# Nyrox/raymond

Measured on AMD Instinct MI355X. Metric: Msamples/s (whole node) + achieved HBM GB/s, 1920x1080 @ 500spp 5-bounce, higher is better.
Workload: dtype f64

## Files before the change

### raymond_amd/csrc/api.cpp

```cpp
#define RMD_WITH_HIP 1
#include <algorithm>
#include <cmath>
#include <limits>
#include <cstdio>
#include <cstdlib>
#include <cstring>
#include <new>

#include "internal.hpp"
#include "launch.hpp"

using rmd::bind;

namespace {
thread_local std::string tl_last_error;

rmd_status context_create(int32_t device, hipStream_t stream, bool own_stream, rmd_context **out) {
	if (!out) return rmd::fail(nullptr, RMD_ERR_INVALID_ARGUMENT, "rmd_context_create: null out pointer");
	*out = nullptr;
	int count = 0;
	hipError_t e = hipGetDeviceCount(&count);
	if (e != hipSuccess || count <= 0)
		return rmd::fail(nullptr, RMD_ERR_NO_DEVICE, std::string("no HIP device: ") + (e != hipSuccess ? hipGetErrorString(e) : "device count is 0"));
	if (device < 0 || device >= count) return rmd::fail(nullptr, RMD_ERR_INVALID_ARGUMENT, "rmd_context_create: device ordinal out of range");
// ... 580 lines not shown
		if (k > sample_count / 4u) k = sample_count / 4u;
		may_buffer_unsplit = false;
	} else if (n_wave_tiles != 0) {
		const uint32_t waves_per_slot = has_grid ? 256u : 24u;
		k = (waves_per_slot * ctx->wave_slots + n_wave_tiles - 1u) / n_wave_tiles;
		if (has_grid && k < 2u) k = 2u;
		uint32_t min_samples = has_grid ? (sample_count <= rmd::kChainMaxSamples && ctx->tunable[RMD_TUNE_CHAIN_ITEMS] != 1 ? 2u : rmd::kSplitMinSamplesGrid) : 64u;
		if (ctx->tunable[RMD_TUNE_SPLIT_MIN_SAMPLES] > 0) min_samples = (uint32_t)std::min<int64_t>(ctx->tunable[RMD_TUNE_SPLIT_MIN_SAMPLES], 1 << 20);
		if (k > sample_count / min_samples) k = sample_count / min_samples;
		if (has_grid && k < 2u && sample_count >= 4u && ctx->tunable[RMD_TUNE_SPLIT_MIN_SAMPLES] <= 0) k = 2u;
	}
	if (k > 64u) k = 64u;
	while (k > 1u && (uint64_t)n_wave_tiles * k > 0x7FFFFFFFull) k--;
	if (k < 2u) k = 1u;
	if (buffered) *buffered = k > 1u || may_buffer_unsplit;
	return k;
}

static rmd_status render_tiles_async_impl(rmd_context *ctx, const rmd_scene *scene, const rmd_camera *camera, const rmd_settings *settings,
                                          const rmd_tile_rect *tiles, uint32_t n_tiles, double *accum_dev, double *accum_sq_dev) {
	if (rmd_status s = bind(ctx)) return s;
	if (rmd_status s = check_render_args(ctx, scene, camera, settings)) return s;
	if (!accum_dev || (n_tiles && !tiles)) return rmd::fail(ctx, RMD_ERR_INVALID_ARGUMENT, "rmd_render_tiles: null tiles/accum pointer");
	if (rmd_status s = prepare_wave_tiles(ctx, camera, tiles, n_tiles)) return s;
	if (settings->bounce_limit == 0u) {
		RMD_HIP(ctx, hipEventRecord(ctx->ev_start, ctx->stream));
		RMD_HIP(ctx, hipEventRecord(ctx->ev_stop, ctx->stream));
		ctx->timed = true;
		return RMD_OK;
	}
	rmd::RenderParams P = rmd::make_params(ctx, scene, camera, settings);
	P.n_work = ctx->n_wave_tiles;
	if (P.debug_flags & 24u) {
		RMD_HIP(ctx, ctx->debug_counters.grow(40 * sizeof(unsigned long long)));
		RMD_HIP(ctx, hipMemsetAsync(ctx->debug_counters.as<void>(), 0, 40 * sizeof(unsigned long long), ctx->stream));
		P.debug_counters = ctx->debug_counters.as<unsigned long long>();
	}
	bool buffered = false;
	uint32_t split = choose_split(ctx, scene->n_grids != 0, P.n_work, P.sample_count, &buffered);
	const bool persistent = ctx->tunable[RMD_TUNE_LAUNCH_FORM] != 1;
	if (persistent) RMD_HIP(ctx, ctx->work_counter.grow(256));
	uint32_t per_pass = P.sample_count;
	if (buffered) {
		const size_t bytes_per_sample = (size_t)P.n_work * 64u * rmd::kSampleStride * sizeof(double);
		size_t cap;
		if (ctx->tunable[RMD_TUNE_SCRATCH_CAP_MB] > 0) cap = (size_t)ctx->tunable[RMD_TUNE_SCRATCH_CAP_MB] << 20;
		else {
			size_t free_b = 0, total_b = 0;
			RMD_HIP(ctx, hipMemGetInfo(&free_b, &total_b));
			cap = (free_b + ctx->sample_buf.bytes()) / 8;
		}
		if (bytes_per_sample * per_pass > cap) per_pass = (uint32_t)(cap / bytes_per_sample);
		const uint64_t sectors_per_sample = (uint64_t)P.n_work * 64u;
		if (sectors_per_sample * per_pass > 0xFFFFFFFFull) per_pass = (uint32_t)(0xFFFFFFFFull / sectors_per_sample);
		if (per_pass < 8u) per_pass = 8u;
		if (per_pass > P.sample_count) per_pass = P.sample_count;
		if (sectors_per_sample * per_pass > 0xFFFFFFFFull) split = 1u, buffered = false, per_pass = P.sample_count;
		while (buffered && bytes_per_sample * per_pass > ctx->sample_buf.bytes()) {
			rmd::DeviceBuffer fresh;
			const hipError_t e = fresh.alloc(bytes_per_sample * per_pass);
			if (e == hipSuccess) {
				ctx->sample_buf = std::move(fresh);
				break;
			}
			(void)hipGetLastError();
			if (e != hipErrorOutOfMemory) return rmd::fail(ctx, RMD_ERR_HIP, std::string("hipMalloc(sample scratch): ") + hipGetErrorString(e));
			if (per_pass <= 8u) {
				split = 1u, buffered = false, per_pass = P.sample_count;
// ... 22 lines not shown
			RMD_HIP(ctx, hipMemsetAsync(ctx->work_counter.as<void>(), 0, sizeof(uint32_t), ctx->stream));
			Q.work_counter = ctx->work_counter.as<uint32_t>();
		}
		if (persistent_pass && buffered && scene->n_grids != 0u && ctx->tunable[RMD_TUNE_PATH_QUEUES] != 1) {
			const size_t wave_bytes = rmd::path_queue_bytes_host(rmd::kQueuePaths), need = wave_bytes * ctx->wave_slots;
			if (ctx->queue_buf.bytes() < need) {
				const hipError_t qe = (ctx->debug_flags & 256u) ? hipErrorOutOfMemory : ctx->queue_buf.grow(need);
				if (qe == hipSuccess) {
					RMD_HIP(ctx, hipMemsetAsync(ctx->queue_buf.as<void>(), 0, need, ctx->stream));
				} else {
					(void)hipGetLastError();
					if (qe != hipErrorOutOfMemory) return rmd::fail(ctx, RMD_ERR_HIP, std::string("hipMalloc(path queues): ") + hipGetErrorString(qe));
				}
			}
			if (ctx->queue_buf.bytes()) Q.queue_buf = ctx->queue_buf.as<unsigned char>(), Q.queue_wave_bytes = (uint32_t)wave_bytes, Q.queue_paths = rmd::kQueuePaths;
		}
		if (buffered && scene->n_grids == 0) {
			RMD_HIP(ctx, ctx->tile_done.grow((size_t)P.n_work * sizeof(uint32_t)));
			RMD_HIP(ctx, hipMemsetAsync(ctx->tile_done.as<void>(), 0, (size_t)P.n_work * sizeof(uint32_t), ctx->stream));
			Q.tile_done = ctx->tile_done.as<uint32_t>();
		}
		rmd::LaunchShape shape;
		RMD_HIP(ctx, rmd::launch_render_tiles(ctx->stream, Q, scene->d_objects, scene->d_grids, ctx->wave_tiles.as<rmd::WaveTile>(), accum_dev, persistent_pass ? ctx->n_cus : 0u, &shape,
		                                      accum_sq_dev));
		ctx->last_launch.passes++, ctx->last_launch.split_k = Q.split_k, ctx->last_launch.buffered = Q.buffered;
		ctx->last_launch.persistent = shape.persistent, ctx->last_launch.waves_per_workgroup = shape.waves_per_wg;
		ctx->last_launch.queued = shape.queued;
		ctx->last_launch.chained = shape.chained;
		if (settings->sample_count == 0) break;
	}
	RMD_HIP(ctx, hipEventRecord(ctx->ev_stop, ctx->stream));
	ctx->timed = true;
	if (P.debug_flags & 24u) {
		unsigned long long h[40];
		RMD_HIP(ctx, hipMemcpyAsync(h, ctx->debug_counters.as<void>(), sizeof(h), hipMemcpyDeviceToHost, ctx->stream));
		RMD_HIP(ctx, hipStreamSynchronize(ctx->stream));
		if ((P.debug_flags & 16u) && ctx->last_launch.queued) {
			static const char *kinds[3] = {"GEN  ", "SHADE", "WALK "};
			for (int k = 0; k < 3; k++)
				std::fprintf(stderr, "[rmd queued stamps, cycles] %s trips=%llu fetch=%llu make_ray=%llu simple=%llu walk=%llu ray_push=%llu classify=%llu stores=%llu\n", kinds[k], h[k * 8 + 7],
				             h[k * 8 + 0], h[k * 8 + 1], h[k * 8 + 2], h[k * 8 + 3], h[k * 8 + 4], h[k * 8 + 5], h[k * 8 + 6]);
			std::fprintf(stderr, "[rmd queued stamps, cycles] inside the walks: init=%llu stepping=%llu entry_wait=%llu scan=%llu (chunk search+load+test)=%llu hits=%llu tail=%llu\n",
			             h[24], h[25], h[26], h[27], h[29], h[30], h[31]);
		} else if (P.debug_flags & 16u)
			std::fprintf(stderr, "[rmd stamps, cycles] wave_total=%llu next_ray=%llu simple=%llu walk=%llu classify=%llu | walk: init=%llu stepping=%llu entry_wait=%llu scan=%llu (chunk search+load+test)=%llu hits=%llu tail=%llu\n",
			             h[0], h[1], h[2], h[3], h[4], h[8], h[9], h[10], h[11], h[13], h[14], h[15]);
		else
			std::fprintf(stderr, "[rmd debug] walk_calls=%llu walkers=%llu calls_with_walkers=%llu rounds=%llu wave_steps=%llu lane_steps=%llu test_rounds=%llu tests=%llu chunks=%llu | main_iterations=%llu live_lanes=%llu lanes_with_ray=%llu | stepping iterations with <= 4 / 8 / 16 lanes: %llu / %llu / %llu, with <= 8 lanes while tests wait: %llu\n",
			             h[0], h[1], h[2], h[3], h[4], h[5], h[6], h[8], h[9], h[10], h[11], h[12], h[7], h[13], h[14], h[15]);
		if ((P.debug_flags & 16u) == 0u)
			std::fprintf(stderr, "[rmd debug] sphere pre-test: pairs passed=%llu full chunks=%llu | pairs dropped that pass the reference's test (flag 64; must be 0)=%llu\n", h[17], h[18], h[16]);
		if ((P.debug_flags & 16u) == 0u && (P.debug_flags & 512u))
			std::fprintf(stderr, "[rmd debug] primary candidates: lanes checked=%llu sphere turns left out=%llu trips with two axis pairs left out=%llu | cleared spheres that register a hit (must be 0)=%llu closest hits that differ from the full visit's (must be 0)=%llu\n",
			             h[32], h[35], h[36], h[33], h[34]);
		if ((P.debug_flags & 16u) == 0u && ctx->last_launch.queued)
			std::fprintf(stderr, "[rmd debug] path queues: rays pushed=%llu (of them walks put aside=%llu) rays held in their lanes=%llu hits pushed=%llu hits held in their lanes=%llu\n", h[19], h[22], h[23], h[20], h[21]);
	}
	return RMD_OK;
}

rmd_status rmd_render_tiles_async(rmd_context *ctx, const rmd_scene *scene, const rmd_camera *camera, const rmd_settings *settings,
                                  const rmd_tile_rect *tiles, uint32_t n_tiles, double *accum_dev) {
	return rmd::guarded(ctx, "rmd_render_tiles", [&] { return render_tiles_async_impl(ctx, scene, camera, settings, tiles, n_tiles, accum_dev, nullptr); });
}

rmd_status rmd_render_tiles_moments_async(rmd_context *ctx, const rmd_scene *scene, const rmd_camera *camera, const rmd_settings *settings,
                                          const rmd_tile_rect *tiles, uint32_t n_tiles, double *accum_dev, double *accum_sq_dev) {
	if (accum_sq_dev != nullptr && accum_sq_dev == accum_dev)
		return rmd::fail(ctx, RMD_ERR_INVALID_ARGUMENT, "rmd_render_tiles_moments: accum_sq_dev must not alias accum_dev");
	return rmd::guarded(ctx, "rmd_render_tiles_moments",
	                    [&] { return render_tiles_async_impl(ctx, scene, camera, settings, tiles, n_tiles, accum_dev, accum_sq_dev); });
}

rmd_status rmd_context_set_tunable(rmd_context *ctx, uint32_t key, int64_t value) {
	if (!ctx) return rmd::fail(nullptr, RMD_ERR_INVALID_ARGUMENT, "rmd_context_set_tunable: null context");
	if (key >= RMD_TUNE_COUNT || value < 0) return rmd::fail(ctx, RMD_ERR_INVALID_ARGUMENT, "rmd_context_set_tunable: unknown key or negative value");
	if (key == RMD_TUNE_LAUNCH_FORM && value > 2) return rmd::fail(ctx, RMD_ERR_INVALID_ARGUMENT, "rmd_context_set_tunable: launch form is 0 .. 2");
	ctx->tunable[key] = value;
	return RMD_OK;
}
rmd_status rmd_context_get_tunable(const rmd_context *ctx, uint32_t key, int64_t *out_value) {
	if (!ctx || !out_value || key >= RMD_TUNE_COUNT) return rmd::fail(nullptr, RMD_ERR_INVALID_ARGUMENT, "rmd_context_get_tunable: bad argument");
	*out_value = ctx->tunable[key];
	return RMD_OK;
}

rmd_status rmd_context_memory_info(rmd_context *ctx, uint64_t *out_free_bytes, uint64_t *out_total_bytes) {
// ... 294 lines not shown
```

### raymond_amd/csrc/device_core.hpp

```cpp
#pragma once
#include <hip/hip_runtime.h>
#include <stdint.h>

#include "device_types.hpp"

#define RMD_DEV __device__ __forceinline__
#ifndef RMD_OPT_BITOP3
#if defined(__gfx950__) || !defined(__HIP_DEVICE_COMPILE__)
#define RMD_OPT_BITOP3 1
#else
#define RMD_OPT_BITOP3 0
#endif
#endif
#define RMD_GLOBAL __attribute__((address_space(1)))
template <class T>
__device__ __forceinline__ const RMD_GLOBAL T *as_global(const T *p) {
	return (const RMD_GLOBAL T *)p;
}

namespace rmd {

struct V3 {
	double x, y, z;
};
// ... 337 lines not shown
	st = sqrt64((1.0 - sr) * (1.0 + sr));
}

RMD_DEV void cosine_hemisphere(double r1, double r2, V3 &dir, double &pdf) {
	double sr = sqrt64(r1);
	double phi = 2.0 * kPi * r2;
	pdf = sr;
	double st, ct, sp, cp;
	hemisphere_sincos(sr, st, ct);
	sincos_cw(phi, sp, cp);
	dir = mk(st * cp, ct, st * sp);
}
RMD_DEV V3 importance_sample_ggx(V3 reflect, double roughness, double r1, double r2) {
	double a = roughness * roughness;
	double phi = 2.0 * kPi * r1;
	double theta = a * sqrt64(r2 / (1.0 - r2));
	double st, ct, sp, cp;
	sincos_cw(theta, st, ct);
	sincos_cw(phi, sp, cp);
	V3 h = mk(st * cp, ct, st * sp);
	V3 tg, bt;
	onb(reflect, tg, bt);
	return normalize(mat3_mul(tg, reflect, bt, h));
}

RMD_DEV double pow5(double x) {
	const double x2 = x * x;
	const double x4 = x2 * x2;
	return x4 * x;
}
RMD_DEV V3 sel(bool c, V3 a, V3 b) { return mk(c ? a.x : b.x, c ? a.y : b.y, c ? a.z : b.z); }

#define RMD_UNDEF(v) asm volatile("" : "=v"(v));
struct NextRayShadeIn {
	V3 normal, frag, color;
	double roughness, metal;
};
RMD_DEV void next_ray(const RenderParams &P, bool do_shade, bool do_prim, const NextRayShadeIn &in, V3 cam_pos, uint32_t prim_x, uint32_t prim_y, Rng &rng,
                      V3 &ro, V3 &rd, V3 &T) {
	const bool gen = do_shade || do_prim;
	double u_first, u_second;
	RMD_UNDEF(u_first) RMD_UNDEF(u_second)
	const double r = (double)rng.lobe_bits * (1.0 / 4194304.0);
	if (gen) {
		uint32_t w0, w1, w2, w3;
		philox4x32_10(rng.pixel, rng.sample, rng.block, 0u, P.key0, P.key1, w0, w1, w2, w3);
		rng.block++;
		u_first = Rng::to_unit(w0, w1), u_second = Rng::to_unit(w2, w3);
		rng.lobe_bits = Rng::spare22(w0, w2);
	}
	V3 pre, view, f0;
	RMD_UNDEF(pre.x) RMD_UNDEF(pre.y) RMD_UNDEF(pre.z) RMD_UNDEF(view.x) RMD_UNDEF(view.y) RMD_UNDEF(view.z) RMD_UNDEF(f0.x) RMD_UNDEF(f0.y) RMD_UNDEF(f0.z)
	bool diffuse = false;
	double prob_d, pdf_d;
	RMD_UNDEF(prob_d) RMD_UNDEF(pdf_d)
	if (do_shade) {
		const V3 normal = in.normal;
		view = normalize(cam_pos - in.frag);
		f0 = mk(lerp(0.04, in.color.x, in.metal), lerp(0.04, in.color.y, in.metal), lerp(0.04, in.color.z, in.metal));
		const double r1 = u_first, r2 = u_second;
		prob_d = lerp(0.5, 0.0, in.metal);
		diffuse = r < prob_d;
		double phi, st, ct, sp, cp;
		V3 axis;
		double root_arg = r1;
		if (!diffuse) root_arg = div_lean(r2, 1.0 - r2);
		const double root = sqrt64(root_arg);
		if (diffuse) {
			hemisphere_sincos(root, st, ct);
			phi = 2.0 * kPi * r2;
			pdf_d = root;
			axis = normal;
		} else {
			const double a = in.roughness * in.roughness;
			phi = 2.0 * kPi * r1;
			sincos_cw(a * root, st, ct);
			axis = normalize(-view - 2.0 * (-dot(view, normal) * normal));
		}
		sincos_cw(phi, sp, cp);
		const V3 local = mk(st * cp, ct, st * sp);
		V3 tg, bt;
		onb(axis, tg, bt);
		pre = mat3_mul(tg, axis, bt, local);
	}
	if (do_prim) {
		const double x = (double)prim_x + (u_first - 0.5);
		const double y = (double)prim_y + (u_second - 0.5);
		const double sx = P.inv_width == P.inv_width ? div_by(x + 0.5, P.width, P.inv_width) : (x + 0.5) / P.width;
		const double sy = P.inv_height == P.inv_height ? div_by(y + 0.5, P.height, P.inv_height) : (y + 0.5) / P.height;
		pre = mk((2.0 * sx - 1.0) * P.tan_half_fov * P.aspect, (1.0 - 2.0 * sy) * P.tan_half_fov, 1.0);
	}
	V3 sw = pre;
	if (gen) sw = normalize(pre);
	if (do_prim) {
		ro = cam_pos, rd = sw;
// ... 9 lines not shown
		V3 vec;
		double N, Dn;
		if (diffuse) {
			const V3 diffuse_part = (mk(1.0, 1.0, 1.0) - F) * (1.0 - in.metal);
			vec = hadamard(diffuse_part, in.color);
			N = fmax(n_dot_sw, 0.0);
			Dn = prob_d * pdf_d;
		} else {
			const double a2 = in.roughness * in.roughness;
			const double ndh = dot(normal, halfway);
			const double den = (ndh * ndh) * (a2 - 1.0) + 1.0;
			const double Dd = fmax(kPi * den * den, 1e-7);
			const double k = (in.roughness * in.roughness) / 8.0;
			const double n_dot_v = dot(normal, view);
			const double g1n = fmax(n_dot_v, 0.0), g2n = fmax(n_dot_sw, 0.0);
			const double g1d = g1n * (1.0 - k) + k, g2d = g2n * (1.0 - k) + k;
			const double denominator = 4.0 * n_dot_v * n_dot_sw + 0.001;
			const double hv4 = 4.0 * h_dot_v;
			vec = F;
			N = (((a2 * g1n) * g2n) * n_dot_sw) * hv4;
			Dn = (((g1d * g2d) * denominator) * (1.0 - prob_d)) * (a2 * ndh + 0.0001 * (Dd * hv4));
		}
		const V3 wgt = vec * (N * fast_rcp(Dn));
		T = hadamard(T, wgt);
		ro = in.frag + normal * (diffuse ? scalar_const(0.00001) : scalar_const(0.0001));
		rd = sw;
	}
}
RMD_DEV void shade(const RenderParams &P, V3 normal, V3 frag, V3 color, double roughness, double metal, V3 cam_pos, Rng &rng, V3 &ro, V3 &rd, V3 &T) {
	NextRayShadeIn in{normal, frag, color, roughness, metal};
	next_ray(P, true, false, in, cam_pos, 0u, 0u, rng, ro, rd, T);
}

RMD_DEV void primary_ray(const RenderParams &P, uint32_t xi, uint32_t yi, double u0, double u1, V3 &ro, V3 &rd) {
	double x = (double)xi + (u0 - 0.5);
	double y = (double)yi + (u1 - 0.5);
	const double sx = P.inv_width == P.inv_width ? div_by(x + 0.5, P.width, P.inv_width) : (x + 0.5) / P.width;
	const double sy = P.inv_height == P.inv_height ? div_by(y + 0.5, P.height, P.inv_height) : (y + 0.5) / P.height;
	double px = (2.0 * sx - 1.0) * P.tan_half_fov * P.aspect;
	double py = (1.0 - 2.0 * sy) * P.tan_half_fov;
	ro = ld3(P.cam_pos);
	rd = normalize(mk(px, py, 1.0));
}
RMD_DEV bool thin_lens_from_pinhole(const RenderParams &P, V3 po, V3 pd, Rng &rng, V3 &ro, V3 &rd);
RMD_DEV bool primary_ray_dof(const RenderParams &P, uint32_t xi, uint32_t yi, Rng &rng, V3 &ro, V3 &rd) {
	double u0, u1;
	rng.next2(P.key0, P.key1, u0, u1);
	V3 po, pd;
	primary_ray(P, xi, yi, u0, u1, po, pd);
	return thin_lens_from_pinhole(P, po, pd, rng, ro, rd);
}
RMD_DEV bool thin_lens_from_pinhole(const RenderParams &P, V3 po, V3 pd, Rng &rng, V3 &ro, V3 &rd) {
	V3 pos = ld3(P.cam_pos);
	V3 start = pos;
	for (int guard = 0; guard < 4096; guard++) {
		double r1, r2;
		rng.next2(P.key0, P.key1, r1, r2);
		r1 = r1 * 2.0 - 1.0, r2 = r2 * 2.0 - 1.0;
		start = mk(pos.x + r1 * P.aperture_radius, pos.y + r2 * P.aperture_radius, pos.z);
		if (dist(start, pos) < P.aperture_radius) break;
	}
	V3 fp_origin = pos + mk(0.0, 0.0, 1.0) * P.focal_length;
	double t;
	if (!plane_intersect(fp_origin, mk(0.0, 0.0, -1.0), po, pd, t)) return false;
	V3 end = pos + t * pd;
	ro = start;
// ... 6 lines not shown
```

### raymond_amd/csrc/launch.hpp

```cpp
#pragma once
#include <hip/hip_runtime_api.h>
#include <stddef.h>
#include <stdint.h>

#include "../../include/raymond_hip.h"
#include "denoise_host.hpp"
#include "device_types.hpp"

#define RMD_PATH_STRIDE 17
#define RMD_MAX_BOUNCE_LIMIT_DEV 16u

namespace rmd {

enum ProbeOp {
	PROBE_PHILOX = 0,
	PROBE_UNIFORM,
	PROBE_SPHERE_INTERSECT,
	PROBE_SPHERE_NORMAL,
	PROBE_PLANE_INTERSECT,
	PROBE_AABB_INTERSECT,
	PROBE_TRIANGLE_INTERSECT,
	PROBE_TRIANGLE_NORMAL,
	PROBE_ONB,
	PROBE_COSINE_HEMISPHERE,
	PROBE_SAMPLE_GGX,
	PROBE_GGX_DISTRIBUTION,
	PROBE_GEOMETRY_SMITH,
	PROBE_FRESNEL_SCHLICK,
	PROBE_PRIMARY_RAY,
	PROBE_ELEMENTARY,
	PROBE_PRETEST_PAIR,
	PROBE_OP_COUNT
};

constexpr size_t kLdsBudgetBytes = 160u * 1024u;
constexpr size_t kMaskBudgetBytes = 48u * 1024u;
constexpr uint32_t kSampleStride = 4;
constexpr uint32_t kWalkBatchDefault = 32;
constexpr uint32_t kSplitMinSamplesGrid = 4;
constexpr uint32_t kSortedMinSamples = 128;
constexpr uint32_t kChainMaxSamples = 0x7FFFFFFF;
constexpr uint32_t kWalkCutDefault = 7;
constexpr double kMaxRoughness = 512.0;
constexpr double kMinRoughness = 1e-12;
constexpr uint32_t kGridWavesPerWg = 4;
constexpr uint32_t kPersistWavesPerWg = 16;
constexpr uint32_t kGridPersistWavesPerWg = 16;
constexpr uint32_t kSortSlots = 120;
constexpr uint32_t kSortedWavesPerWg = 16;
constexpr size_t kSortPoolBytes = 84u * kSortSlots;
constexpr size_t kWaveHeadBytes = 16u;
struct LaunchShape {
	uint32_t persistent = 0, waves_per_wg = 0, queued = 0, resident_waves = 0, chained = 0;
};
struct LaunchPlan {
	uint32_t persistent = 0, queued = 0, chained = 0, moments = 0, waves_per_wg = 0, workgroups = 0;
	size_t wave_lds = 0, lds = 0;
};
LaunchPlan plan_render_launch(int mode, bool grid, uint32_t n_objects, uint32_t mask_words_total, bool queues, bool persist, bool chain_items, bool moments,
                              uint32_t n_waves, uint32_t n_cus);
void render_lds_sizes(int mode, bool grid, uint64_t out[8]);
constexpr uint32_t kQueuePaths = 256;
inline size_t path_queue_bytes_host(uint32_t cap) { return (size_t)cap * (9u * 8u + 13u * 8u + 4u * 4u + 9u * 4u); }
static_assert(kQueuePaths >= 192u && kQueuePaths % 64u == 0u, "two stacks short of a full trip + the 64 paths of a generation trip");
size_t render_lds_bytes(uint32_t n_objects, uint32_t mask_words_total, uint32_t waves_per_wg);
hipError_t launch_render_tiles(hipStream_t stream, const RenderParams &P, const DevObject *objs, const DevGrid *grids,
                               const WaveTile *wave_tiles, double *accum, uint32_t n_cus = 0, LaunchShape *shape = nullptr, double *accum_sq = nullptr);
hipError_t launch_tile_error(hipStream_t stream, const double *accum, const double *accum_sq, const rmd_tile_rect *rects, uint32_t n_rects, uint32_t W,
                             uint32_t sample_count, double floor, double *out);
constexpr uint32_t kDenoiseTile = 16;
constexpr double kDenoiseEps = 1e-10;
constexpr uint32_t kDenoiseMaxRadius = 12, kDenoiseMaxPatch = 4;
constexpr uint32_t kDenoiseMaxCandidates = (uint32_t)RMD_DENOISE_MAX_CANDIDATES, kDenoiseMaxSelectWindow = 5;
constexpr int kDenoiseFeat = (int)RMD_FEATURE_CHANNELS;
size_t denoise_lds_bytes(uint32_t tile_width, uint32_t radius, uint32_t patch_radius);
uint32_t denoise_tile_width(uint32_t radius, uint32_t patch_radius);
struct DenoiseInput {
	const double *accum_a, *accum_sq_a, *accum_b, *accum_sq_b, *feat, *feat_sq;
	const rmd_tile_rect *rects;
	const uint32_t *counts_a, *counts_b, *counts_f;
	uint32_t n_rects, count_image_columns, W, H;
};
struct DenoiseWeights {
// ... 39 lines not shown
```

### raymond_amd/csrc/render_kernel.hpp

```cpp
#pragma once
#include <hip/hip_runtime.h>

#include "device_core.hpp"
#include "grid_walk.hpp"
#include "launch.hpp"
#include "primary_candidates.hpp"
#include "scene_split.hpp"

namespace rmd {

struct alignas(16) PathId {
	uint32_t px[64];
	uint32_t smp[64];
	uint32_t sector[64];
};
__host__ __device__ inline size_t wave_lds_bytes(uint32_t n_grids) { return kWaveHeadBytes + (n_grids ? sizeof(WalkScratch) + 64u * 3u * sizeof(double) + sizeof(WalkCarry) + sizeof(PathId) : 0); }

RMD_DEV uint32_t work_item_of_block(uint32_t b, uint32_t nb) {
	(void)nb;
	return b;
}

RMD_DEV void report_fault(const RenderParams &P, uint32_t code, uint32_t detail) {
	if ((threadIdx.x & 63u) == 0u) {
		if (P.fault != nullptr) {
			__hip_atomic_fetch_or(P.fault, code, __ATOMIC_RELAXED, __HIP_MEMORY_SCOPE_SYSTEM);
			__hip_atomic_store(P.fault + 1, detail, __ATOMIC_RELAXED, __HIP_MEMORY_SCOPE_SYSTEM);
			__hip_atomic_fetch_add(P.fault + 2, 1u, __ATOMIC_RELAXED, __HIP_MEMORY_SCOPE_SYSTEM);
		}
		if (P.work_counter != nullptr) __hip_atomic_fetch_or(P.work_counter, kWorkCounterPoison, __ATOMIC_RELAXED, __HIP_MEMORY_SCOPE_AGENT);
	}
}
constexpr uint32_t kTripBoundPerPair = RMD_MAX_BOUNCE_LIMIT_DEV + 4u;
constexpr uint32_t kStallBound = 1u << 18;

template <bool GRID>
RMD_DEV int scene_intersect_wave(const DevObject *__restrict__ objs, uint32_t n_objects, const DevGrid *__restrict__ grids,
                                 const uint32_t *lds_masks, WalkScratch &scr, bool want, V3 ro, V3 rd, double &t_best, uint32_t &sub_best,
// ... 452 lines not shown
				} else {
					intersect_grids<false>(objs, Pt.n_objects, grids, lds_masks, scr, want && waiting, ro, rd, part_t, part_obj, part_sub, Pt.debug_flags, Pt.debug_counters, 0u, nullptr, nullptr, 0u,
					                       Pt.grid_mask);
					waiting = false;
				}
			}
			RMD_TSTAMP(tt_walk)
			complete = want && !waiting;
			t = part_t, oi = part_obj, sub = part_sub;
		} else {
			oi = scene_intersect_wave<false>(objs, Pt.n_objects, grids, lds_masks, scr, want, ro, rd, t, sub, Pt.axis_pairs, Pt.debug_flags, Pt.debug_counters, false, Pt.visit_mask);
			complete = want;
		}
	}

#if RMD_DIAG
	if (tstamp && lane == 0) {
		atomicAdd(&P.debug_counters[0], __builtin_amdgcn_s_memtime() - tt_begin), atomicAdd(&P.debug_counters[1], tt_b);
		atomicAdd(&P.debug_counters[2], tt_simple), atomicAdd(&P.debug_counters[3], tt_walk), atomicAdd(&P.debug_counters[4], tt_class);
	}
#endif
#undef RMD_TSTAMP
	if constexpr (to_buffer && !GRID) finish_sample_range(P, tile, wt, lane, out);
	if (writes && !to_buffer && !acc_in_memory) {
		out[out_index + 0] = acc.x;
		out[out_index + 1] = acc.y;
		out[out_index + 2] = acc.z;
		if constexpr (MOM && !acc_in_memory) out_sq[out_index + 0] = acc_sq.x, out_sq[out_index + 1] = acc_sq.y, out_sq[out_index + 2] = acc_sq.z;
	}
}

constexpr int kSortObjPrio = 1;
struct alignas(16) HitStack {
	double frag[3][kSortSlots], normal[3][kSortSlots], T[3][kSortSlots];
	uint32_t state[kSortSlots];
	uint32_t lobe_bits[kSortSlots];
	uint32_t item[kSortSlots];
};
static_assert(kSortSlots >= 72u && kSortSlots <= 512u && kSortSlots % 8u == 0u, "a generation trip needs room for 64 more hits");
static_assert(sizeof(HitStack) == kSortPoolBytes, "launch.hpp: kSortPoolBytes");
using SortPool = HitStack;

RMD_DEV void item_candidates(KernargWords kernarg_params, WaveTile tile, const DevObject *__restrict__ objs, const DevObject *lobjs, uint32_t *sets) {
	const uint32_t lane = threadIdx.x & 63u;
	KernargWords src = kernarg_params;
	asm volatile("" : "+s"(src));
	unsigned long long w[sizeof(RenderParams) / 8];
#pragma unroll
	for (unsigned i = 0; i < sizeof(RenderParams) / 8; i++) w[i] = src[i];
	RenderParams P;
	__builtin_memcpy(&P, w, sizeof(P));
	unsigned long long visit = P.visit_mask;
	uint32_t pairs = P.axis_pairs;
	if (P.primary_cull != 0u) {
		CullCamera cc;
		cc.pos[0] = P.cam_pos[0], cc.pos[1] = P.cam_pos[1], cc.pos[2] = P.cam_pos[2];
		cc.width = P.width, cc.height = P.height, cc.aspect = P.aspect, cc.tan_half_fov = P.tan_half_fov;
		const TileCone cone = primary_tile_cone(cc, tile.x0, tile.y0, tile.w, tile.h);
		const DevObject &o = lobjs[lane < P.n_objects ? lane : 0u];
		const double centre[3] = {o.origin[0], o.origin[1], o.origin[2]};
		const bool cleared = lane < P.n_objects && o.geometry_kind == 1u && primary_sphere_cleared(cone, cc, centre, o.radius);
		visit &= ~__ballot(cleared);
		const AxisWalls *walls = reinterpret_cast<const AxisWalls *>(objs + P.n_objects);
		const AxisWalls w3[3] = {walls[0], walls[1], walls[2]};
		pairs = primary_pairs_kept(cone, cc, w3, P.axis_pairs);
	}
	if (lane == 0u) sets[0] = pairs, sets[1] = (uint32_t)visit, sets[2] = (uint32_t)(visit >> 32);
	__builtin_amdgcn_fence(__ATOMIC_RELEASE, "wavefront");
	__builtin_amdgcn_wave_barrier();
	__builtin_amdgcn_fence(__ATOMIC_ACQUIRE, "wavefront");
}
#define RMD_UNDEF3(v) RMD_UNDEF(v.x) RMD_UNDEF(v.y) RMD_UNDEF(v.z)
template <bool MOM = false>
RMD_DEV void render_wave_sorted(const RenderParams &P, KernargWords kernarg_params, const DevObject *__restrict__ objs, const DevGrid *__restrict__ grids,
                                const void *__restrict__ work, double *__restrict__ out, const DevObject *lobjs, unsigned char *wave_lds, uint32_t work_item,
                                double *__restrict__ out_sq = nullptr) {
	const uint32_t lane = threadIdx.x & 63u;
	HitStack &stack = *reinterpret_cast<HitStack *>(wave_lds);
	WalkScratch *no_scratch = nullptr;
	const uint32_t wt = work_item / P.split_k, part = work_item % P.split_k;
	const bool have = wt < P.n_work;
	const WaveTile tile = reinterpret_cast<const WaveTile *>(work)[have ? wt : 0];
	const uint32_t per_part = (P.sample_count + P.split_k - 1u) / P.split_k;
	const uint32_t s_lo = part * per_part < P.sample_count ? part * per_part : P.sample_count;
	const uint32_t s_hi = s_lo + per_part < P.sample_count ? s_lo + per_part : P.sample_count;
	const uint32_t pool_first = s_lo, pool_items = have ? (s_hi - s_lo) * 64u : 0u;
	if (P.bounce_limit == 0u) return;
	const V3 cam_pos = ld3(P.cam_pos);

	uint32_t *item_sets = reinterpret_cast<uint32_t *>(wave_lds + sizeof(HitStack)) + 1;
	item_candidates(kernarg_params, tile, objs, lobjs, item_sets);

	uint32_t n_hit = 0, next_item = 0;
	unsigned long long trips_left = (unsigned long long)pool_items * kTripBoundPerPair + 64ull;
#if RMD_DIAG
	if (P.debug_flags & 32u) trips_left = 1ull;
#endif
	for (;;) {
		KernargWords src = kernarg_params;
		asm volatile("" : "+s"(src));
		unsigned long long w[sizeof(RenderParams) / 8];
#pragma unroll
		for (unsigned i = 0; i < sizeof(RenderParams) / 8; i++) w[i] = src[i];
		RenderParams Pt;
		__builtin_memcpy(&Pt, w, sizeof(Pt));

		if (RMD_UNLIKELY(trips_left-- == 0ull)) {
			report_fault(Pt, kFaultSortedTripLoop, work_item);
			n_hit = 0u, next_item = pool_items;
		}
		const bool items_left = next_item < pool_items;
		if (n_hit == 0u && !items_left) break;
		const bool shade_trip = !items_left || n_hit > kSortSlots - 64u;
		bool active;
		uint32_t item = 0, depth = 1;
		Rng rng;
		rng.block = 0u, rng.lobe_bits = 0u;
		V3 ro, rd, T;
		RMD_UNDEF3(ro) RMD_UNDEF3(rd) RMD_UNDEF3(T)
		bool failed = false;
		unsigned long long turns = Pt.visit_mask;
		uint32_t pairs = Pt.axis_pairs;
		if (shade_trip) {
			const uint32_t n = n_hit < 64u ? n_hit : 64u;
			active = lane < n;
			const uint32_t e = active ? n_hit - n + lane : 0u;
			n_hit -= n;
			const uint32_t st = stack.state[e];
			item = stack.item[e];
			const uint32_t lb = stack.lobe_bits[e];
			rng.block = st >> 16, rng.lobe_bits = lb & 0x3FFFFFu;
			depth = lb >> 24;
			const DevObject &o = lobjs[active ? (st & 0xFFFFu) : 0u];
			T = mk(stack.T[0][e], stack.T[1][e], stack.T[2][e]);
			const V3 normal = mk(stack.normal[0][e], stack.normal[1][e], stack.normal[2][e]);
			const V3 frag = mk(stack.frag[0][e], stack.frag[1][e], stack.frag[2][e]);
			const uint32_t x = tile.x0 + (item & 7u), y = tile.y0 + ((item >> 3) & 7u);
			rng.pixel = y * Pt.W + x, rng.sample = Pt.sample_begin + pool_first + (item >> 6);
			{
				shade(Pt, normal, frag, ld3(o.color), o.roughness, o.metalness, cam_pos, rng, ro, rd, T);
				depth++;
				const bool black = Pt.end_black_paths != 0u && T.x == 0.0 && T.y == 0.0 && T.z == 0.0;
				failed = active && (depth > Pt.bounce_limit || black);
			}
		} else {
			item = next_item + lane;
			next_item += 64u;
			active = item < pool_items && (item & 7u) < tile.w && ((item >> 3) & 7u) < tile.h;
			const uint32_t x = tile.x0 + (item & 7u), y = tile.y0 + ((item >> 3) & 7u);
			rng.pixel = y * Pt.W + x, rng.sample = Pt.sample_begin + pool_first + (item >> 6);
			T = mk(1.0, 1.0, 1.0);
			{
				double u0, u1;
				rng.next2(Pt.key0, Pt.key1, u0, u1);
				primary_ray(Pt, x, y, u0, u1, ro, rd);
				if (Pt.use_dof) failed = active && !thin_lens_from_pinhole(Pt, ro, rd, rng, ro, rd);
			}
			pairs = (uint32_t)__builtin_amdgcn_readfirstlane((int)item_sets[0]);
			turns = (unsigned long long)(uint32_t)__builtin_amdgcn_readfirstlane((int)item_sets[1]) | (unsigned long long)(uint32_t)__builtin_amdgcn_readfirstlane((int)item_sets[2]) << 32;
		}
		const bool want = active && !failed;
		double t = 0.0;
		uint32_t sub = 0;
		__builtin_amdgcn_s_setprio(kSortObjPrio);
		const int oi = scene_intersect_wave<false>(objs, Pt.n_objects, grids, nullptr, *no_scratch, want, ro, rd, t, sub, pairs, 0u, nullptr, false, turns);
		__builtin_amdgcn_s_setprio(0);
#if RMD_DIAG
		if ((Pt.debug_flags & 512u) && (Pt.debug_flags & 8u) && Pt.debug_counters && !shade_trip) {
			double t_full = 0.0;
			uint32_t sub_full = 0;
			const int oi_full = scene_intersect_wave<false>(objs, Pt.n_objects, grids, nullptr, *no_scratch, want, ro, rd, t_full, sub_full, Pt.axis_pairs, 0u, nullptr, false, Pt.visit_mask);
			const bool differs = want && (oi_full != oi || __builtin_bit_cast(unsigned long long, t_full) != __builtin_bit_cast(unsigned long long, t));
			unsigned long long wrong = 0ull;
			const unsigned long long dropped = Pt.visit_mask & ~turns;
			for (unsigned long long m = dropped; m != 0ull; m &= m - 1ull) {
				const DevObject &o = objs[__builtin_ctzll(m)];
				double ts;
				wrong += (unsigned long long)__popcll(__ballot(want && sphere_test_flat(ld3(o.origin), o.radius, ro, rd, ts)));
			}
			const unsigned long long dm = __ballot(differs), wm = __ballot(want);
			if (lane == 0u) {
				atomicAdd(&Pt.debug_counters[32], (unsigned long long)__popcll(wm)), atomicAdd(&Pt.debug_counters[33], wrong);
				atomicAdd(&Pt.debug_counters[34], (unsigned long long)__popcll(dm)), atomicAdd(&Pt.debug_counters[35], (unsigned long long)__popcll(dropped));
				atomicAdd(&Pt.debug_counters[36], pairs != Pt.axis_pairs ? 1ull : 0ull);
			}
		}
#endif
		bool terminal = failed, park = false, emitted = false;
		V3 frag, normal;
		RMD_UNDEF3(frag) RMD_UNDEF3(normal)
		if (want) {
			if (oi < 0) {
				terminal = true;
			} else {
				const DevObject &o = lobjs[oi];
				frag = ro + rd * t;
				if (o.material_kind == 2u) {
					emitted = true;
					terminal = true;
				} else {
					if (o.geometry_kind == 0u) normal = ld3(o.normal);
					else normal = normalize(frag - ld3(o.origin));
					const double probe_sum = ((normal.x + normal.y) + normal.z) + ((frag.x + frag.y) + frag.z);
					const bool finite_inputs = __builtin_fabs(probe_sum) < __builtin_inf();
					const bool black_bounce = Pt.end_black_paths != 0u && (o.flags & kObjBlackDiffuse) != 0u && rng.lobe_bits < (1u << 21);
					if (((depth == Pt.bounce_limit && Pt.shade_last_depth == 0u) || black_bounce) && finite_inputs) terminal = true;
					else park = true;
				}
			}
		}
		if (active && terminal) {
			V3 L = mk(0.0, 0.0, 0.0);
			if (emitted) L = ld3(lobjs[oi].color);
			L = hadamard(T, L);
			RMD_GLOBAL double *dst = (RMD_GLOBAL double *)Pt.sample_buf + (((size_t)wt * Pt.sample_count + pool_first + (item >> 6)) * 64u + (item & 63u)) * kSampleStride;
			store_sample(dst, L);
		}
		{
			const unsigned long long pm = __ballot(park);
			const uint32_t e = n_hit + __builtin_amdgcn_mbcnt_hi((uint32_t)(pm >> 32), __builtin_amdgcn_mbcnt_lo((uint32_t)pm, 0u));
			if (park) {
				stack.frag[0][e] = frag.x, stack.frag[1][e] = frag.y, stack.frag[2][e] = frag.z;
				stack.normal[0][e] = normal.x, stack.normal[1][e] = normal.y, stack.normal[2][e] = normal.z;
				stack.T[0][e] = T.x, stack.T[1][e] = T.y, stack.T[2][e] = T.z;
				stack.state[e] = (uint32_t)oi | (rng.block << 16);
				stack.lobe_bits[e] = rng.lobe_bits | (depth << 24), stack.item[e] = item;
			}
			n_hit += (uint32_t)__popcll(pm);
			__builtin_amdgcn_fence(__ATOMIC_RELEASE, "wavefront");
			__builtin_amdgcn_wave_barrier();
			__builtin_amdgcn_fence(__ATOMIC_ACQUIRE, "wavefront");
		}
	}
	finish_sample_range<MOM>(P, tile, wt, lane, out, out_sq);
}

struct PathQueues {
	RMD_GLOBAL double *hit_d;
	RMD_GLOBAL double *ray_d;
	RMD_GLOBAL uint32_t *hit_w;
	RMD_GLOBAL uint32_t *ray_w;
	uint32_t cap;
};
constexpr uint32_t kRayCarried = 1u << 23;
__host__ __device__ inline size_t path_queue_bytes(uint32_t cap) { return (size_t)cap * (9u * 8u + 13u * 8u + 4u * 4u + 9u * 4u); }
RMD_DEV uint32_t sample_of_sector(const RenderParams &P, uint32_t sector) {
	const uint32_t a = sector >> 6, q = (uint32_t)__umul64hi((unsigned long long)a, P.sample_magic);
	return P.sample_begin + (P.sample_magic != 0ull ? a - q * P.sample_count : 0u);
}
constexpr uint32_t kQueuedTripBoundPerPath = 2u * RMD_MAX_BOUNCE_LIMIT_DEV + 4u;
constexpr size_t kQueuedSideBytes = 64u * (3u * sizeof(double) + 4u * sizeof(uint32_t));
constexpr size_t kQueuedDiagBytes = RMD_DIAG ? 24u * sizeof(unsigned long long) : 0u;
__host__ __device__ inline size_t queued_wave_lds_bytes() { return sizeof(WalkScratch) + sizeof(WalkCarry) + kQueuedSideBytes + kQueuedDiagBytes + kWaveHeadBytes; }

template <class T>
RMD_DEV T qld(const RMD_GLOBAL T *p) {
	return *p;
}
template <class T, class U>
RMD_DEV void qst(RMD_GLOBAL T *p, U v) {
	*p = (T)v;
// ... 515 lines not shown
```

Measured before the change: 25410.

## Split sorted hit stack into diffuse and GGX lobe stacks for coherent shading

Parked hits are now split by BSDF lobe, which is chosen early from the stored lobe bits. They go into a two-ended LDS stack, diffuse from the bottom and GGX from the top, and each shade trip takes up to 64 hits of a single lobe. Shading then runs a specialised template per lobe, so a wave no longer diverges across both lobe branches. Normals are no longer kept in LDS but recomputed from the object at shade time, which shrinks each slot from 84 to 60 bytes and lets 168 slots fit in the same pool. The cost is extra normal work and an object load per shade, plus shade trips that can run with fewer full lanes when one lobe is scarce.

```diff
diff --git a/raymond_amd/csrc/api.cpp b/raymond_amd/csrc/api.cpp
--- a/raymond_amd/csrc/api.cpp
+++ b/raymond_amd/csrc/api.cpp
@@ -636,8 +636,8 @@
 	rmd::RenderParams P = rmd::make_params(ctx, scene, camera, settings);
 	P.n_work = ctx->n_wave_tiles;
 	if (P.debug_flags & 24u) {
-		RMD_HIP(ctx, ctx->debug_counters.grow(40 * sizeof(unsigned long long)));
-		RMD_HIP(ctx, hipMemsetAsync(ctx->debug_counters.as<void>(), 0, 40 * sizeof(unsigned long long), ctx->stream));
+		RMD_HIP(ctx, ctx->debug_counters.grow(48 * sizeof(unsigned long long)));
+		RMD_HIP(ctx, hipMemsetAsync(ctx->debug_counters.as<void>(), 0, 48 * sizeof(unsigned long long), ctx->stream));
 		P.debug_counters = ctx->debug_counters.as<unsigned long long>();
 	}
 	bool buffered = false;
@@ -726,7 +726,7 @@
 	RMD_HIP(ctx, hipEventRecord(ctx->ev_stop, ctx->stream));
 	ctx->timed = true;
 	if (P.debug_flags & 24u) {
-		unsigned long long h[40];
+		unsigned long long h[48];
 		RMD_HIP(ctx, hipMemcpyAsync(h, ctx->debug_counters.as<void>(), sizeof(h), hipMemcpyDeviceToHost, ctx->stream));
 		RMD_HIP(ctx, hipStreamSynchronize(ctx->stream));
 		if ((P.debug_flags & 16u) && ctx->last_launch.queued) {
@@ -747,6 +747,9 @@
 		if ((P.debug_flags & 16u) == 0u && (P.debug_flags & 512u))
 			std::fprintf(stderr, "[rmd debug] primary candidates: lanes checked=%llu sphere turns left out=%llu trips with two axis pairs left out=%llu | cleared spheres that register a hit (must be 0)=%llu closest hits that differ from the full visit's (must be 0)=%llu\n",
 			             h[32], h[35], h[36], h[33], h[34]);
+		if ((P.debug_flags & 16u) == 0u && ctx->last_launch.buffered && scene->n_grids == 0u)
+			std::fprintf(stderr, "[rmd debug] lobe trips: diffuse trips=%llu diffuse hits shaded=%llu ggx trips=%llu ggx hits shaded=%llu | hits parked: diffuse=%llu ggx=%llu\n", h[37], h[38], h[39],
+			             h[40], h[41], h[42]);
 		if ((P.debug_flags & 16u) == 0u && ctx->last_launch.queued)
 			std::fprintf(stderr, "[rmd debug] path queues: rays pushed=%llu (of them walks put aside=%llu) rays held in their lanes=%llu hits pushed=%llu hits held in their lanes=%llu\n", h[19], h[22], h[23], h[20], h[21]);
 	}
diff --git a/raymond_amd/csrc/device_core.hpp b/raymond_amd/csrc/device_core.hpp
--- a/raymond_amd/csrc/device_core.hpp
+++ b/raymond_amd/csrc/device_core.hpp
@@ -393,6 +393,11 @@
 RMD_DEV V3 sel(bool c, V3 a, V3 b) { return mk(c ? a.x : b.x, c ? a.y : b.y, c ? a.z : b.z); }
 
 #define RMD_UNDEF(v) asm volatile("" : "=v"(v));
+RMD_DEV double lobe_uniform(uint32_t lobe_bits) { return (double)lobe_bits * (1.0 / 4194304.0); }
+RMD_DEV bool bounce_is_diffuse(double r, double metal, double &prob_d) {
+	prob_d = lerp(0.5, 0.0, metal);
+	return r < prob_d;
+}
 struct NextRayShadeIn {
 	V3 normal, frag, color;
 	double roughness, metal;
@@ -402,7 +407,7 @@
 	const bool gen = do_shade || do_prim;
 	double u_first, u_second;
 	RMD_UNDEF(u_first) RMD_UNDEF(u_second)
-	const double r = (double)rng.lobe_bits * (1.0 / 4194304.0);
+	const double r = lobe_uniform(rng.lobe_bits);
 	if (gen) {
 		uint32_t w0, w1, w2, w3;
 		philox4x32_10(rng.pixel, rng.sample, rng.block, 0u, P.key0, P.key1, w0, w1, w2, w3);
@@ -420,8 +425,7 @@
 		view = normalize(cam_pos - in.frag);
 		f0 = mk(lerp(0.04, in.color.x, in.metal), lerp(0.04, in.color.y, in.metal), lerp(0.04, in.color.z, in.metal));
 		const double r1 = u_first, r2 = u_second;
-		prob_d = lerp(0.5, 0.0, in.metal);
-		diffuse = r < prob_d;
+		diffuse = bounce_is_diffuse(r, in.metal, prob_d);
 		double phi, st, ct, sp, cp;
 		V3 axis;
 		double root_arg = r1;
@@ -497,6 +501,69 @@
 	next_ray(P, true, false, in, cam_pos, 0u, 0u, rng, ro, rd, T);
 }
 
+template <bool DIFFUSE>
+RMD_DEV void shade_lobe(const RenderParams &P, V3 normal, V3 frag, V3 color, double roughness, double metal, V3 cam_pos, Rng &rng, V3 &ro, V3 &rd, V3 &T) {
+	uint32_t w0, w1, w2, w3;
+	philox4x32_10(rng.pixel, rng.sample, rng.block, 0u, P.key0, P.key1, w0, w1, w2, w3);
+	rng.block++;
+	const double r1 = Rng::to_unit(w0, w1), r2 = Rng::to_unit(w2, w3);
+	rng.lobe_bits = Rng::spare22(w0, w2);
+	const V3 view = normalize(cam_pos - frag);
+	const V3 f0 = mk(lerp(0.04, color.x, metal), lerp(0.04, color.y, metal), lerp(0.04, color.z, metal));
+	const double prob_d = lerp(0.5, 0.0, metal);
+	double phi, st, ct, sp, cp, pdf_d = 0.0;
+	V3 axis;
+	if constexpr (DIFFUSE) {
+		const double root = sqrt64(r1);
+		hemisphere_sincos(root, st, ct);
+		phi = 2.0 * kPi * r2;
+		pdf_d = root;
+		axis = normal;
+	} else {
+		const double root = sqrt64(div_lean(r2, 1.0 - r2));
+		const double a = roughness * roughness;
+		phi = 2.0 * kPi * r1;
+		sincos_cw(a * root, st, ct);
+		axis = normalize(-view - 2.0 * (-dot(view, normal) * normal));
+	}
+	sincos_cw(phi, sp, cp);
+	const V3 local = mk(st * cp, ct, st * sp);
+	V3 tg, bt;
+	onb(axis, tg, bt);
+	const V3 sw = normalize(mat3_mul(tg, axis, bt, local));
+	const double n_dot_sw = dot(normal, sw);
+	const V3 halfway = normalize_for_weight(sw + view);
+	const double h_dot_v = dot(halfway, view);
+	const double fc = DIFFUSE ? fmax(h_dot_v, 0.0) : h_dot_v;
+	const V3 F = f0 + (mk(1.0, 1.0, 1.0) - f0) * pow5(1.0 - fc);
+	V3 vec;
+	double N, Dn;
+	if constexpr (DIFFUSE) {
+		const V3 diffuse_part = (mk(1.0, 1.0, 1.0) - F) * (1.0 - metal);
+		vec = hadamard(diffuse_part, color);
+		N = fmax(n_dot_sw, 0.0);
+		Dn = prob_d * pdf_d;
+	} else {
+		const double a2 = roughness * roughness;
+		const double ndh = dot(normal, halfway);
+		const double den = (ndh * ndh) * (a2 - 1.0) + 1.0;
+		const double Dd = fmax(kPi * den * den, 1e-7);
+		const double k = (roughness * roughness) / 8.0;
+		const double n_dot_v = dot(normal, view);
+		const double g1n = fmax(n_dot_v, 0.0), g2n = fmax(n_dot_sw, 0.0);
+		const double g1d = g1n * (1.0 - k) + k, g2d = g2n * (1.0 - k) + k;
+		const double denominator = 4.0 * n_dot_v * n_dot_sw + 0.001;
+		const double hv4 = 4.0 * h_dot_v;
+		vec = F;
+		N = (((a2 * g1n) * g2n) * n_dot_sw) * hv4;
+		Dn = (((g1d * g2d) * denominator) * (1.0 - prob_d)) * (a2 * ndh + 0.0001 * (Dd * hv4));
+	}
+	const V3 wgt = vec * (N * fast_rcp(Dn));
+	T = hadamard(T, wgt);
+	ro = frag + normal * (DIFFUSE ? scalar_const(0.00001) : scalar_const(0.0001));
+	rd = sw;
+}
+
 RMD_DEV void primary_ray(const RenderParams &P, uint32_t xi, uint32_t yi, double u0, double u1, V3 &ro, V3 &rd) {
 	double x = (double)xi + (u0 - 0.5);
 	double y = (double)yi + (u1 - 0.5);
diff --git a/raymond_amd/csrc/launch.hpp b/raymond_amd/csrc/launch.hpp
--- a/raymond_amd/csrc/launch.hpp
+++ b/raymond_amd/csrc/launch.hpp
@@ -46,9 +46,9 @@
 constexpr uint32_t kGridWavesPerWg = 4;
 constexpr uint32_t kPersistWavesPerWg = 16;
 constexpr uint32_t kGridPersistWavesPerWg = 16;
-constexpr uint32_t kSortSlots = 120;
+constexpr uint32_t kSortSlots = 168;
 constexpr uint32_t kSortedWavesPerWg = 16;
-constexpr size_t kSortPoolBytes = 84u * kSortSlots;
+constexpr size_t kSortPoolBytes = 60u * kSortSlots;
 constexpr size_t kWaveHeadBytes = 16u;
 struct LaunchShape {
 	uint32_t persistent = 0, waves_per_wg = 0, queued = 0, resident_waves = 0, chained = 0;
diff --git a/raymond_amd/csrc/lobe_trips.hpp b/raymond_amd/csrc/lobe_trips.hpp
--- /dev/null
+++ b/raymond_amd/csrc/lobe_trips.hpp
@@ -0,0 +1,34 @@
+#pragma once
+#include <stdint.h>
+
+#if defined(__HIP__)
+#define RMD_LOBE_HD __host__ __device__ inline
+#else
+#define RMD_LOBE_HD inline
+#endif
+
+namespace rmd {
+
+enum : uint32_t { kTripDone = 0, kTripGenerate = 1, kTripShadeDiffuse = 2, kTripShadeGgx = 3 };
+struct LobeTrip {
+	uint32_t kind;
+	uint32_t lanes;
+};
+RMD_LOBE_HD LobeTrip lobe_trip_rule(uint32_t n_d, uint32_t n_g, bool items_left, uint32_t slots) {
+	LobeTrip t;
+	if (items_left && n_d + n_g + 64u <= slots) {
+		t.kind = kTripGenerate, t.lanes = 64u;
+	} else if (n_d + n_g == 0u) {
+		t.kind = kTripDone, t.lanes = 0u;
+	} else {
+		const bool diffuse = n_d >= n_g;
+		const uint32_t n = diffuse ? n_d : n_g;
+		t.kind = diffuse ? kTripShadeDiffuse : kTripShadeGgx, t.lanes = n < 64u ? n : 64u;
+	}
+	return t;
+}
+RMD_LOBE_HD unsigned long long lobe_trip_bound(uint32_t pool_items, uint32_t per_pair) { return (unsigned long long)pool_items * per_pair + 64ull; }
+RMD_LOBE_HD uint32_t lobe_pop_first(bool diffuse, uint32_t n_d, uint32_t n_g, uint32_t lanes, uint32_t slots) { return diffuse ? n_d - lanes : slots - n_g; }
+RMD_LOBE_HD uint32_t lobe_push_entry(bool diffuse, uint32_t n_d, uint32_t n_g, uint32_t rank, uint32_t slots) { return diffuse ? n_d + rank : slots - 1u - n_g - rank; }
+
+}
diff --git a/raymond_amd/csrc/render_kernel.hpp b/raymond_amd/csrc/render_kernel.hpp
--- a/raymond_amd/csrc/render_kernel.hpp
+++ b/raymond_amd/csrc/render_kernel.hpp
@@ -4,6 +4,7 @@
 #include "device_core.hpp"
 #include "grid_walk.hpp"
 #include "launch.hpp"
+#include "lobe_trips.hpp"
 #include "primary_candidates.hpp"
 #include "scene_split.hpp"
 
@@ -522,7 +523,7 @@
 
 constexpr int kSortObjPrio = 1;
 struct alignas(16) HitStack {
-	double frag[3][kSortSlots], normal[3][kSortSlots], T[3][kSortSlots];
+	double frag[3][kSortSlots], T[3][kSortSlots];
 	uint32_t state[kSortSlots];
 	uint32_t lobe_bits[kSortSlots];
 	uint32_t item[kSortSlots];
@@ -581,8 +582,8 @@
 	uint32_t *item_sets = reinterpret_cast<uint32_t *>(wave_lds + sizeof(HitStack)) + 1;
 	item_candidates(kernarg_params, tile, objs, lobjs, item_sets);
 
-	uint32_t n_hit = 0, next_item = 0;
-	unsigned long long trips_left = (unsigned long long)pool_items * kTripBoundPerPair + 64ull;
+	uint32_t n_d = 0, n_g = 0, next_item = 0;
+	unsigned long long trips_left = lobe_trip_bound(pool_items, kTripBoundPerPair);
 #if RMD_DIAG
 	if (P.debug_flags & 32u) trips_left = 1ull;
 #endif
@@ -597,11 +598,11 @@
 
 		if (RMD_UNLIKELY(trips_left-- == 0ull)) {
 			report_fault(Pt, kFaultSortedTripLoop, work_item);
-			n_hit = 0u, next_item = pool_items;
-		}
-		const bool items_left = next_item < pool_items;
-		if (n_hit == 0u && !items_left) break;
-		const bool shade_trip = !items_left || n_hit > kSortSlots - 64u;
+			n_d = 0u, n_g = 0u, next_item = pool_items;
+		}
+		const LobeTrip trip = lobe_trip_rule(n_d, n_g, next_item < pool_items, kSortSlots);
+		if (trip.kind == kTripDone) break;
+		const bool shade_trip = trip.kind != kTripGenerate;
 		bool active;
 		uint32_t item = 0, depth = 1;
 		Rng rng;
@@ -612,23 +613,32 @@
 		unsigned long long turns = Pt.visit_mask;
 		uint32_t pairs = Pt.axis_pairs;
 		if (shade_trip) {
-			const uint32_t n = n_hit < 64u ? n_hit : 64u;
+			const bool lobe_d = trip.kind == kTripShadeDiffuse;
+			const uint32_t n = trip.lanes;
 			active = lane < n;
-			const uint32_t e = active ? n_hit - n + lane : 0u;
-			n_hit -= n;
+			const uint32_t e = lobe_pop_first(lobe_d, n_d, n_g, n, kSortSlots) + (active ? lane : 0u);
+			if (lobe_d) n_d -= n;
+			else n_g -= n;
+#if RMD_DIAG
+			if ((Pt.debug_flags & 8u) && Pt.debug_counters && lane == 0u)
+				atomicAdd(&Pt.debug_counters[lobe_d ? 37 : 39], 1ull), atomicAdd(&Pt.debug_counters[lobe_d ? 38 : 40], (unsigned long long)n);
+#endif
 			const uint32_t st = stack.state[e];
 			item = stack.item[e];
 			const uint32_t lb = stack.lobe_bits[e];
 			rng.block = st >> 16, rng.lobe_bits = lb & 0x3FFFFFu;
 			depth = lb >> 24;
-			const DevObject &o = lobjs[active ? (st & 0xFFFFu) : 0u];
+			const DevObject &o = lobjs[st & 0xFFFFu];
 			T = mk(stack.T[0][e], stack.T[1][e], stack.T[2][e]);
-			const V3 normal = mk(stack.normal[0][e], stack.normal[1][e], stack.normal[2][e]);
 			const V3 frag = mk(stack.frag[0][e], stack.frag[1][e], stack.frag[2][e]);
+			V3 normal;
+			if (o.geometry_kind == 0u) normal = ld3(o.normal);
+			else normal = normalize(frag - ld3(o.origin));
 			const uint32_t x = tile.x0 + (item & 7u), y = tile.y0 + ((item >> 3) & 7u);
 			rng.pixel = y * Pt.W + x, rng.sample = Pt.sample_begin + pool_first + (item >> 6);
 			{
-				shade(Pt, normal, frag, ld3(o.color), o.roughness, o.metalness, cam_pos, rng, ro, rd, T);
+				if (lobe_d) shade_lobe<true>(Pt, normal, frag, ld3(o.color), o.roughness, o.metalness, cam_pos, rng, ro, rd, T);
+				else shade_lobe<false>(Pt, normal, frag, ld3(o.color), o.roughness, o.metalness, cam_pos, rng, ro, rd, T);
 				depth++;
 				const bool black = Pt.end_black_paths != 0u && T.x == 0.0 && T.y == 0.0 && T.z == 0.0;
 				failed = active && (depth > Pt.bounce_limit || black);
@@ -677,8 +687,9 @@
 		}
 #endif
 		bool terminal = failed, park = false, emitted = false;
-		V3 frag, normal;
-		RMD_UNDEF3(frag) RMD_UNDEF3(normal)
+		bool park_d = false;
+		V3 frag;
+		RMD_UNDEF3(frag)
 		if (want) {
 			if (oi < 0) {
 				terminal = true;
@@ -689,13 +700,18 @@
 					emitted = true;
 					terminal = true;
 				} else {
-					if (o.geometry_kind == 0u) normal = ld3(o.normal);
-					else normal = normalize(frag - ld3(o.origin));
-					const double probe_sum = ((normal.x + normal.y) + normal.z) + ((frag.x + frag.y) + frag.z);
-					const bool finite_inputs = __builtin_fabs(probe_sum) < __builtin_inf();
 					const bool black_bounce = Pt.end_black_paths != 0u && (o.flags & kObjBlackDiffuse) != 0u && rng.lobe_bits < (1u << 21);
-					if (((depth == Pt.bounce_limit && Pt.shade_last_depth == 0u) || black_bounce) && finite_inputs) terminal = true;
-					else park = true;
+					park = true;
+					if ((depth == Pt.bounce_limit && Pt.shade_last_depth == 0u) || black_bounce) {
+						V3 normal;
+						if (o.geometry_kind == 0u) normal = ld3(o.normal);
+						else normal = normalize(frag - ld3(o.origin));
+						const double probe_sum = ((normal.x + normal.y) + normal.z) + ((frag.x + frag.y) + frag.z);
+						const bool finite_inputs = __builtin_fabs(probe_sum) < __builtin_inf();
+						if (finite_inputs) terminal = true, park = false;
+					}
+					double prob_d;
+					park_d = bounce_is_diffuse(lobe_uniform(rng.lobe_bits), o.metalness, prob_d);
 				}
 			}
 		}
@@ -707,16 +723,21 @@
 			store_sample(dst, L);
 		}
 		{
-			const unsigned long long pm = __ballot(park);
-			const uint32_t e = n_hit + __builtin_amdgcn_mbcnt_hi((uint32_t)(pm >> 32), __builtin_amdgcn_mbcnt_lo((uint32_t)pm, 0u));
+			const unsigned long long pm_d = __ballot(park && park_d), pm_g = __ballot(park && !park_d);
+			const uint32_t rank_d = __builtin_amdgcn_mbcnt_hi((uint32_t)(pm_d >> 32), __builtin_amdgcn_mbcnt_lo((uint32_t)pm_d, 0u));
+			const uint32_t rank_g = __builtin_amdgcn_mbcnt_hi((uint32_t)(pm_g >> 32), __builtin_amdgcn_mbcnt_lo((uint32_t)pm_g, 0u));
+			const uint32_t e = lobe_push_entry(park_d, n_d, n_g, park_d ? rank_d : rank_g, kSortSlots);
 			if (park) {
 				stack.frag[0][e] = frag.x, stack.frag[1][e] = frag.y, stack.frag[2][e] = frag.z;
-				stack.normal[0][e] = normal.x, stack.normal[1][e] = normal.y, stack.normal[2][e] = normal.z;
 				stack.T[0][e] = T.x, stack.T[1][e] = T.y, stack.T[2][e] = T.z;
 				stack.state[e] = (uint32_t)oi | (rng.block << 16);
 				stack.lobe_bits[e] = rng.lobe_bits | (depth << 24), stack.item[e] = item;
 			}
-			n_hit += (uint32_t)__popcll(pm);
+			n_d += (uint32_t)__popcll(pm_d), n_g += (uint32_t)__popcll(pm_g);
+#if RMD_DIAG
+			if ((Pt.debug_flags & 8u) && Pt.debug_counters && lane == 0u)
+				atomicAdd(&Pt.debug_counters[41], (unsigned long long)__popcll(pm_d)), atomicAdd(&Pt.debug_counters[42], (unsigned long long)__popcll(pm_g));
+#endif
 			__builtin_amdgcn_fence(__ATOMIC_RELEASE, "wavefront");
 			__builtin_amdgcn_wave_barrier();
 			__builtin_amdgcn_fence(__ATOMIC_ACQUIRE, "wavefront");
```

Measured after the change: 25720, median of 6. +1.2%, better.
